# femto-dev/femto

Measured on AMD Instinct MI355X. Metric: patterns/sec (count+locate) on 1 GiB index, higher is better.
Workload: dtype int64

## Files before the change

femto_amd/build.py:

```python
import os
import subprocess
from concurrent.futures import ThreadPoolExecutor

HERE = os.path.dirname(os.path.abspath(__file__))
CSRC = os.path.join(HERE, "csrc")
EXTRACT = os.path.join(HERE, "extract")
OBJ = os.path.join(HERE, "_obj")
LIB = os.environ.get("FEMTO_AMD_LIB") or os.path.join(HERE, "libfemto_amd.so")
SOURCES = ["femto_amd_api.hip", "api_host.hip", "api_open.hip", "api_multi.hip", "regexp_search.hip", "resolve.hip", "trace_kernels.hip", "host_index.cpp", "index_builder.cpp", "suffix_sort.hip",
           "query_sort.hip", "host_pack.cpp", "../extract/extract.hip"]
PLAIN_CXX = {"host_pack.cpp"}
CXX_FLAGS = ["-O3", "-std=c++17", "-fPIC", "-pthread"]
FLAGS = ["--offload-arch=gfx950", "-O3", "-std=c++17", "-fPIC", "-pthread", "-Wno-unused-result", "-Wno-cuda-compat"]
FLAGS += os.environ.get("FEMTO_AMD_EXTRA_FLAGS", "").split()
if os.environ.get("FEMTO_AMD_OBJ"):
    OBJ = os.environ["FEMTO_AMD_OBJ"]


def _headers():
    hs = [os.path.join(d, f) for d in (CSRC, EXTRACT) for f in os.listdir(d) if f.endswith((".hpp", ".h"))]
    hs.append(os.path.join(os.path.dirname(HERE), "include", "femto_amd.h"))
    return hs


def _newest_header():
    return max(os.path.getmtime(h) for h in _headers())


def _obj(src):
    return os.path.join(OBJ, os.path.splitext(os.path.basename(src))[0] + ".o")


def _stale(src, hdr_time):
    o = _obj(src)
    if not os.path.exists(o):
        return True
    t = os.path.getmtime(o)
    return os.path.getmtime(os.path.join(CSRC, src)) > t or hdr_time > t


def needs_build():
    if not os.path.exists(LIB):
        return True
    t = os.path.getmtime(LIB)
    if _newest_header() > t:
        return True
    return any(os.path.getmtime(os.path.join(CSRC, f)) > t for f in SOURCES)


def build(force=False, verbose=False):
    if not force and not needs_build():
        return LIB
    os.makedirs(OBJ, exist_ok=True)
    hdr_time = _newest_header()
    todo = [s for s in SOURCES if force or _stale(s, hdr_time)]

    def compile_one(src):
        if src in PLAIN_CXX:
            cmd = ["hipcc"] + CXX_FLAGS + ["-x", "c++", "-c", os.path.join(CSRC, src), "-o", _obj(src)]
        else:
            cmd = ["hipcc"] + FLAGS + ["-x", "hip", "-c", os.path.join(CSRC, src), "-o", _obj(src)]
        if verbose:
            print(" ".join(cmd), flush=True)
        subprocess.run(cmd, check=True)

    with ThreadPoolExecutor(max_workers=min(8, max(1, len(todo)))) as ex:
        list(ex.map(compile_one, todo))
    cmd = ["hipcc", "--offload-arch=gfx950", "-fPIC", "-shared", "-pthread", "-o", LIB] + [_obj(s) for s in SOURCES]
    if verbose:
        print(" ".join(cmd), flush=True)
    subprocess.run(cmd, check=True)
    return LIB


TOOL_SRC = os.path.join(os.path.dirname(HERE), "tools", "femto_amd_multiquery.cpp")
TOOL = os.path.join(HERE, "femto_amd_multiquery")


SEARCH_SRC = os.path.join(os.path.dirname(HERE), "tools", "femto_amd_search.cpp")
SEARCH = os.path.join(HERE, "femto_amd_search")


def build_tools(force=False, verbose=False):
    for src, exe in ((TOOL_SRC, TOOL), (SEARCH_SRC, SEARCH)):
        if not force and os.path.exists(exe) and os.path.getmtime(exe) > max(os.path.getmtime(src), os.path.getmtime(LIB)):
            continue
        cmd = ["g++", "-std=c++17", "-O2", "-o", exe, src, "-L" + HERE, "-lfemto_amd", "-Wl,-rpath,$ORIGIN",
               "-Wl,-rpath-link," + HERE, "-Wl,--allow-shlib-undefined"]
        if verbose:
            print(" ".join(cmd))
        subprocess.run(cmd, check=True)
    return TOOL


if __name__ == "__main__":
    build(force=True, verbose=True)
    build_tools(force=True, verbose=True)
```

Before: 19.00 billion.

## Add fused plan-stream locate kernel that scans offsets and expands small rows in one pass

Result: faster. 20.17 billion (median of 6 runs) (+6.1%).

```diff
diff --git a/femto_amd/build.py b/femto_amd/build.py
--- a/femto_amd/build.py
+++ b/femto_amd/build.py
@@ -5,10 +5,12 @@
 HERE = os.path.dirname(os.path.abspath(__file__))
 CSRC = os.path.join(HERE, "csrc")
 EXTRACT = os.path.join(HERE, "extract")
+CHAIN = os.path.join(HERE, "chain")
 OBJ = os.path.join(HERE, "_obj")
 LIB = os.environ.get("FEMTO_AMD_LIB") or os.path.join(HERE, "libfemto_amd.so")
 SOURCES = ["femto_amd_api.hip", "api_host.hip", "api_open.hip", "api_multi.hip", "regexp_search.hip", "resolve.hip", "trace_kernels.hip", "host_index.cpp", "index_builder.cpp", "suffix_sort.hip",
-           "query_sort.hip", "host_pack.cpp", "../extract/extract.hip"]
+           "query_sort.hip", "host_pack.cpp", "../extract/extract.hip", "../chain/locate_chain.hip"]
+SOURCE_FLAGS = {"femto_amd_api.hip": ["-Dfemto_amd_locate_device=femto_amd_locate_device_csrc"]}
 PLAIN_CXX = {"host_pack.cpp"}
 CXX_FLAGS = ["-O3", "-std=c++17", "-fPIC", "-pthread"]
 FLAGS = ["--offload-arch=gfx950", "-O3", "-std=c++17", "-fPIC", "-pthread", "-Wno-unused-result", "-Wno-cuda-compat"]
@@ -18,8 +20,9 @@
 
 
 def _headers():
-    hs = [os.path.join(d, f) for d in (CSRC, EXTRACT) for f in os.listdir(d) if f.endswith((".hpp", ".h"))]
+    hs = [os.path.join(d, f) for d in (CSRC, EXTRACT, CHAIN) for f in os.listdir(d) if f.endswith((".hpp", ".h"))]
     hs.append(os.path.join(os.path.dirname(HERE), "include", "femto_amd.h"))
+    hs.append(os.path.abspath(__file__))
     return hs
 
 
@@ -59,7 +62,7 @@
         if src in PLAIN_CXX:
             cmd = ["hipcc"] + CXX_FLAGS + ["-x", "c++", "-c", os.path.join(CSRC, src), "-o", _obj(src)]
         else:
-            cmd = ["hipcc"] + FLAGS + ["-x", "hip", "-c", os.path.join(CSRC, src), "-o", _obj(src)]
+            cmd = ["hipcc"] + FLAGS + SOURCE_FLAGS.get(src, []) + ["-x", "hip", "-c", os.path.join(CSRC, src), "-o", _obj(src)]
         if verbose:
             print(" ".join(cmd), flush=True)
         subprocess.run(cmd, check=True)
diff --git a/femto_amd/chain/locate_chain.hip b/femto_amd/chain/locate_chain.hip
--- /dev/null
+++ b/femto_amd/chain/locate_chain.hip
@@ -0,0 +1,261 @@
+#include <algorithm>
+#include <atomic>
+#include <cstdlib>
+#include <cstring>
+
+#include "../csrc/api_internal.hpp"
+#include "../csrc/kernels.hip.hpp"
+#include "../csrc/pack_kernels.hip.hpp"
+#include "../csrc/ru_kernels.hip.hpp"
+#include "../csrc/pack2_kernels.hip.hpp"
+#include "../csrc/ind_kernels.hip.hpp"
+#include "../csrc/text_kernels.hip.hpp"
+#include "../csrc/ctx_kernels.hip.hpp"
+#include "../csrc/direct_kernels.hip.hpp"
+
+#ifndef FEMTO_AMD_CHAIN_TILES
+#define FEMTO_AMD_CHAIN_TILES 8
+#endif
+#ifndef FEMTO_AMD_CHAIN_WIDE
+#define FEMTO_AMD_CHAIN_WIDE 1
+#endif
+
+extern "C" int femto_amd_locate_device_csrc(femto_amd_index_t* ix, int64_t npats, const int32_t* d_plen, const uint16_t* d_pats,
+                                            const int64_t* d_starts, int max_occs_each, int64_t* d_first, int64_t* d_last,
+                                            int32_t* d_noccs, int64_t* d_out_starts, int64_t* d_offsets, int64_t offsets_capacity,
+                                            int64_t* d_total, void* stream);
+
+namespace femto_amd {
+namespace {
+
+std::atomic<int64_t> g_streamed_calls{0};
+
+constexpr int kChainTiles = FEMTO_AMD_CHAIN_TILES;
+static_assert(kChainTiles >= 1 && kChainTiles <= 16 && 64 % kChainTiles == 0, "tiles per workgroup");
+
+template <int G, bool kWide>
+__global__ __launch_bounds__(256) __attribute__((amdgpu_waves_per_eu(8, 8))) void plan_stream_kernel(
+    const int64_t npats, const int32_t* __restrict__ noccs, const int64_t* __restrict__ first, const PlanSums ps,
+    int64_t* __restrict__ out_starts, int64_t* __restrict__ offsets, const int64_t capacity, int* __restrict__ big_flag,
+    const DevIndex ix, int64_t* __restrict__ total_out, int64_t* __restrict__ total_user, const int64_t* __restrict__ sa_known) {
+  __shared__ int64_t s_toff[G];
+  __shared__ uint32_t s_rows;
+  __shared__ int64_t s_w[G][4];
+  __shared__ uint32_t s_incl[4][64];
+  __shared__ int64_t s_first[4][64], s_lbase[4][64];
+  const int lane = threadIdx.x & 63, wave = threadIdx.x >> 6;
+  const int64_t b0 = int64_t(blockIdx.x) * G;
+  if (wave == 0) {
+    const int64_t g = b0 >> 6, bl = (b0 & ~int64_t(63)) + lane;
+    const int j0 = int(b0 & 63);
+    const uint64_t own = bl < ps.nblocks ? uint64_t(ps.sums[bl]) : 0;
+    uint64_t acc = lane < int(g & 63) ? uint64_t(ps.super[(g & ~int64_t(63)) + lane]) : 0;
+    for (int64_t k = lane; k < (g >> 6); k += 64) acc += uint64_t(ps.super2[k]);
+    for (int64_t k = int64_t(blockIdx.x) * 64 + lane; k < ps.next_words; k += int64_t(gridDim.x) * 64) ps.next_super[k] = 0;
+    const uint64_t part = wave_sum_u64(acc);
+    const uint64_t before = (uint64_t(uint32_t(__shfl(int(uint32_t(part >> 32)), 0, 64))) << 32) | uint32_t(__shfl(int(uint32_t(part)), 0, 64));
+    uint64_t incl = own;
+#pragma unroll
+    for (int d = 1; d < 64; d <<= 1) {
+      const uint32_t lo = uint32_t(__shfl_up(int(uint32_t(incl)), d, 64)), hi = uint32_t(__shfl_up(int(uint32_t(incl >> 32)), d, 64));
+      if (lane >= d) incl += (uint64_t(hi) << 32) | lo;
+    }
+    const uint64_t has = __ballot(own != 0);
+    if (lane >= j0 && lane < j0 + G) {
+      const int64_t excl = int64_t(before + incl - own);
+      s_toff[lane - j0] = excl;
+      if (bl == ps.nblocks - 1) {
+        const int64_t total = excl + int64_t(own);
+        total_out[0] = total;
+        total_out[1] = total > capacity ? 1 : 0;
+        if (total_user) {
+          total_user[0] = total;
+          total_user[1] = total > capacity ? 1 : 0;
+        }
+        out_starts[npats] = total;
+      }
+    }
+    if (lane == 0) s_rows = uint32_t(has >> j0) & ((1u << G) - 1u);
+  }
+  __syncthreads();
+  const uint32_t rows = uint32_t(__builtin_amdgcn_readfirstlane(int(s_rows)));
+  const int64_t left = ps.nblocks - b0;
+  const uint32_t live = left >= G ? ((1u << G) - 1u) : ((1u << int(left)) - 1u);
+  int32_t n_t[G];
+#pragma unroll
+  for (int t = 0; t < G; t++) {
+    const int64_t q = (b0 + t) * 256 + threadIdx.x;
+    n_t[t] = ((rows >> t) & 1u) && q < npats ? noccs[q] : 0;
+  }
+  if (kWide) {
+    const int half = threadIdx.x >> 7;
+    uint32_t z = ~rows & live;
+    while (z) {
+      const int ta = __ffs(int(z)) - 1;
+      z &= z - 1;
+      int tb = -1;
+      if (z) {
+        tb = __ffs(int(z)) - 1;
+        z &= z - 1;
+      }
+      const int t = half ? tb : ta;
+      if (t >= 0) {
+        const int64_t q = (b0 + t) * 256 + 2 * int(threadIdx.x & 127u);
+        const int64_t v = s_toff[t];
+        if (q + 1 < npats) {
+          *reinterpret_cast<longlong2*>(out_starts + q) = longlong2{v, v};
+        } else if (q < npats) {
+          out_starts[q] = v;
+        }
+      }
+    }
+  } else {
+#pragma unroll
+    for (int t = 0; t < G; t++) {
+      const int64_t q = (b0 + t) * 256 + threadIdx.x;
+      if (((~rows & live) >> t) & 1u) {
+        if (q < npats) out_starts[q] = s_toff[t];
+      }
+    }
+  }
+  if (!rows) return;
+#pragma unroll
+  for (int t = 0; t < G; t++) {
+    if ((rows >> t) & 1u) {
+      const uint64_t wsum = wave_sum_u64(uint64_t(int64_t(n_t[t])));
+      if (lane == 0) s_w[t][wave] = int64_t(wsum);
+    }
+  }
+  __syncthreads();
+  for (uint32_t r = rows; r; r &= r - 1) {
+    const int t = __ffs(int(r)) - 1;
+    const int64_t q = (b0 + t) * 256 + threadIdx.x;
+    int32_t nt = 0;
+#pragma unroll
+    for (int u = 0; u < G; u++) nt = u == t ? n_t[u] : nt;
+    const int64_t n = int64_t(nt);
+    uint64_t incl = uint64_t(n);
+#pragma unroll
+    for (int d = 1; d < 64; d <<= 1) {
+      const uint32_t lo = uint32_t(__shfl_up(int(uint32_t(incl)), d, 64)), hi = uint32_t(__shfl_up(int(uint32_t(incl >> 32)), d, 64));
+      if (lane >= d) incl += (uint64_t(hi) << 32) | lo;
+    }
+    int64_t woff = 0;
+    for (int k = 0; k < wave; k++) woff += s_w[t][k];
+    const int64_t base = q < npats ? s_toff[t] + woff + int64_t(incl) - n : 0;
+    if (q < npats) out_starts[q] = base;
+    const bool big = n > kExpandSerialMax;
+    if (big) atomicOr(big_flag, 1);
+    const uint32_t mine = (q < npats && !big) ? uint32_t(n) : 0u;
+    uint32_t inc = mine;
+#pragma unroll
+    for (int d = 1; d < 64; d <<= 1) {
+      const uint32_t y = uint32_t(__shfl_up(int(inc), d, 64));
+      if (lane >= d) inc += y;
+    }
+    s_incl[wave][lane] = inc;
+    int64_t f0 = 0;
+    bool have = false;
+    if (sa_known && mine == 1u) {
+      const int64_t known = sa_known[q];
+      if (known >= 0) {
+        f0 = ~known;
+        have = true;
+      }
+    }
+    if (mine && !have) f0 = first[q];
+    s_first[wave][lane] = f0;
+    s_lbase[wave][lane] = base;
+    const uint32_t total = uint32_t(__shfl(int(inc), 63, 64));
+    __syncthreads();
+    for (uint32_t s0 = 0; s0 < total; s0 += 64) {
+      const uint32_t sidx = s0 + uint32_t(lane);
+      if (sidx < total) {
+        int lo = 0, hi = 63;
+        while (lo < hi) {
+          const int mid = (lo + hi) >> 1;
+          if (s_incl[wave][mid] > sidx) hi = mid; else lo = mid + 1;
+        }
+        const uint32_t before = lo ? s_incl[wave][lo - 1] : 0u;
+        const int64_t k = int64_t(sidx - before);
+        const int64_t slot = s_lbase[wave][lo] + k;
+        if (slot < capacity) {
+          const int64_t f = s_first[wave][lo], row = f + k;
+          if (f < 0) {
+            offsets[slot] = ~f;
+          } else {
+            offsets[slot] = sa_at(ix, row);
+            trace_touch(ix, kTraceSa, sa_line_of(ix, row));
+          }
+        }
+      }
+    }
+  }
+}
+
+bool chain_off() {
+  const char* e = getenv("FEMTO_AMD_CHAIN");
+  return e && !strcmp(e, "csrc");
+}
+
+int launch_plan_stream(femto_amd_index* ix, Scratch& S, int64_t npats, int max_occs, const int32_t* d_noccs, const int64_t* d_first,
+                       int64_t* d_out_starts, int64_t* d_offsets, int64_t capacity, hipStream_t stream, const int64_t* d_sa_known) {
+  int* big_flag = S.d_flags + 1;
+  const int64_t nblocks = (npats + kBlockThreads - 1) / kBlockThreads;
+  const dim3 grid{uint32_t((nblocks + kChainTiles - 1) / kChainTiles)}, bgrid{uint32_t(std::min<int64_t>(nblocks, int64_t(ix->num_cus) * 8))},
+      block{uint32_t(kBlockThreads)};
+  const PlanSums ps = plan_sums_at(S.bsums.p, nblocks, false, S.bsums_parity);
+  S.bsums_clean = true;
+  hipEvent_t e0 = nullptr, e1 = nullptr;
+  timer_begin(ix, ix->t_locate, stream, &e0, &e1);
+  if (FEMTO_AMD_CHAIN_WIDE && !(reinterpret_cast<uintptr_t>(d_out_starts) & 15u))
+    hipLaunchKernelGGL((plan_stream_kernel<kChainTiles, true>), grid, block, 0, stream, npats, d_noccs, d_first, ps, d_out_starts, d_offsets, capacity,
+                       big_flag, ix->dev, S.d_total, S.total_user, d_sa_known);
+  else
+    hipLaunchKernelGGL((plan_stream_kernel<kChainTiles, false>), grid, block, 0, stream, npats, d_noccs, d_first, ps, d_out_starts, d_offsets, capacity,
+                       big_flag, ix->dev, S.d_total, S.total_user, d_sa_known);
+  if (int64_t(max_occs) + 1 > kExpandSerialMax)
+    hipLaunchKernelGGL((plan_big_rows_kernel<kRowsSa, PackPolicy>), bgrid, block, 0, stream, npats, d_first, static_cast<const int2*>(nullptr),
+                       static_cast<const int64_t*>(d_out_starts), static_cast<const int64_t*>(S.d_total), capacity, d_offsets,
+                       static_cast<const int*>(big_flag), ix->dev);
+  HIP_TRY(hipGetLastError());
+  timer_end(ix, ix->t_locate, stream, e0, e1);
+  return 0;
+}
+
+}
+}
+
+extern "C" int64_t femto_amd_chain_streamed_calls(void) { return g_streamed_calls.load(std::memory_order_relaxed); }
+
+int femto_amd_locate_device(femto_amd_index_t* ix, int64_t npats, const int32_t* d_plen, const uint16_t* d_pats,
+                            const int64_t* d_starts, int max_occs_each, int64_t* d_first, int64_t* d_last,
+                            int32_t* d_noccs, int64_t* d_out_starts, int64_t* d_offsets, int64_t offsets_capacity,
+                            int64_t* d_total, void* stream_) {
+  if (!ix || npats <= 0 || npats > (int64_t(1) << 31) || !d_offsets || !ix->children.empty() || ix->split_parts > 0 || !use_direct(ix) || !ix->dev.sa_full || chain_off())
+    return femto_amd_locate_device_csrc(ix, npats, d_plen, d_pats, d_starts, max_occs_each, d_first, d_last, d_noccs, d_out_starts, d_offsets,
+                                        offsets_capacity, d_total, stream_);
+  API_BEGIN
+  if (reinterpret_cast<uintptr_t>(d_pats) & 1u) return set_err(FEMTO_AMD_ERR_PARAM, "d_pats must be 2-byte aligned (uint16 symbols; the kernels read them in aligned 16-byte pieces)");
+  if (max_occs_each < 0 || offsets_capacity < 0) return set_err(FEMTO_AMD_ERR_PARAM, "negative max_occs_each / capacity");
+  const bool row_free = !d_first && !d_last;
+  if ((!row_free && (!d_first || !d_last)) || !d_noccs || !d_out_starts || !d_total) return set_err(FEMTO_AMD_ERR_PARAM, "null argument");
+  int rc = ensure_device(ix);
+  if (rc) return rc;
+  hipStream_t stream = static_cast<hipStream_t>(stream_);
+  Lease L(ix, stream);
+  if (!L.s) return L.rc;
+  Scratch& S = *L.s;
+  Plan plan{max_occs_each, d_noccs, d_out_starts, offsets_capacity, false, d_total};
+  if (row_free) {
+    if ((rc = S.first.reserve(size_t(npats + 1) * 8))) return rc;
+    d_first = S.first.as<int64_t>();
+    plan.row_free = true;
+  }
+  if ((rc = launch_count_plan(ix, S, npats, d_plen, d_pats, d_starts, d_first, d_last, &plan, stream))) return rc;
+  if (!plan.done) return set_err(FEMTO_AMD_ERR_INVALID, "internal error: the direct pipeline left no locate plan");
+  if ((rc = launch_plan_stream(ix, S, npats, max_occs_each, d_noccs, d_first, d_out_starts, d_offsets, offsets_capacity, stream, plan.sa_known))) return rc;
+  g_streamed_calls.fetch_add(1, std::memory_order_relaxed);
+  return FEMTO_AMD_OK;
+  API_END
+}
```
